# Strong-AI-Lab/ct-vae

Measured on AMD Instinct MI355X. Metric: images/sec/GPU fwd+bwd, 64×64×3 bs=64; recon+KL vs CPU ref, higher is better.
Workload: dtype f32; 1 GPU; VanillaVAE 64x64x3 train step fwd+loss+bwd+Adam (configs/vae.yaml shapes at the batch BASELINE.json's metric names, bs=64, on one MI355X; BASELINE.json configs[1..4] are the `configs` entries); per_gpu_batch=64, global_batch=64, latent_dim=128, parallelism=single, hipgraph=True, allreduce_overlap=False

## Files before the change

### ct-vae_amd/csrc/api.hip

```cpp
#include "../../include/ctvae_hip.h"

#include "common.hpp"
#include "gatlayer.hpp"
#include "glinear.hpp"
#include "pair.hpp"

namespace ctvae {
int launch_tapgemm(const ConvGeom& g, const float* G, const float* W, const float* bias, const float* add,
                   const float* mask, int mask_act, float* S, int act, float* bn_part, float* ws, size_t ws_floats,
                   hipStream_t st, const BnBwdFuse* bnb = nullptr, const InXform* xf = nullptr,
                   const WinoFilters* wf = nullptr, SplitKRaw* raw = nullptr, int out_pix = 0);
bool out_pix_supported(const ConvGeom& g, size_t ws_floats, int out_pix);
bool wino_supported(const ConvGeom& g, size_t ws_floats);
bool wino_enabled();
int wino_set_enabled(int on);
int launch_crop_resize_u8(const unsigned char* img, const long long* rows, float* out, int B, int N, int H, int W, int crop,
                          int S, hipStream_t st);
bool thin_forward_supported(const ConvGeom& g);
bool thin_wgrad_supported(const ConvGeom& g);
int tapgemm_bnb_rows(const ConvGeom& g, size_t ws_floats);
bool img_dgrad_supported(const ConvGeom& g);
void tapgemm_plan(const ConvGeom& g, size_t ws_floats, TapGemmPlan& p);
int launch_wgrad(const ConvGeom& g, const float* X, const float* dY, float* dW, float* dbias, float* ws, size_t ws_bytes,
                 int accumulate, hipStream_t st, const InXform* xf = nullptr, const DyXform* dyx = nullptr);
// ... 265 lines not shown
int ctvae_conv_bn_act_apply_is_separate(int kind, int B, int H, int W, int Ci, int Co, int k, int stride, int pad, int out_pad,
                                        size_t ws_bytes) {
  if (!conv_kind_ok(kind)) return 0;
  ConvGeom g;
  if (conv_geom(g, kind, 0, B, H, W, Ci, Co, k, stride, pad, out_pad)) return 0;
  TapGemmPlan plan;
  tapgemm_plan(g, ws_bytes / sizeof(float), plan);
  return (plan.splitk > 1 && bn_fused_ok(g.B * g.sH * g.sW, Co)) ? 0 : 1;
}

int ctvae_conv_bn_act_forward(int kind, const float* x, const float* w, const float* bias, const float* gamma,
                              const float* beta, float* running_mean, float* running_var, float momentum, float eps,
                              int training, int act, float* y, float* a_out, float* save_mean, float* save_invstd,
                              float* scale_shift_out, int64_t* num_batches_tracked, int B, int H, int W, int Ci, int Co, int k,
                              int stride, int pad, int out_pad, const float* in_scale, const float* in_shift, int in_act,
                              float* ws, size_t ws_bytes, void* stream) {
  long long* nbt = (long long*)num_batches_tracked;
  if (!x || !w || !gamma || !beta || !y || !ws || !conv_kind_ok(kind)) return kErrBadArg;
  if ((in_scale != nullptr) != (in_shift != nullptr)) return kErrBadArg;
  if (in_scale != nullptr && !ctvae_conv_input_transform_supported(kind, B, H, W, Ci, Co, k, stride, pad, out_pad)) return kErrBadArg;
  const InXform xf{in_scale, in_shift, in_act};
  const InXform* xfp = in_scale != nullptr ? &xf : nullptr;
  if (!a_out && !scale_shift_out) return kErrBadArg;
  if (training && (!save_mean || !save_invstd)) return kErrBadArg;
  if (!training && (!running_mean || !running_var)) return kErrBadArg;
  if (Co % 4 != 0) return kErrBadArg;
  ConvGeom g;
  if (conv_geom(g, kind, 0, B, H, W, Ci, Co, k, stride, pad, out_pad)) return kErrBadArg;
  const size_t wsf = ws_bytes / sizeof(float);
  TapGemmPlan plan;
  tapgemm_plan(g, wsf, plan);
  const int R = g.B * g.sH * g.sW;
  if (plan.splitk > 1 || !training) {
    SplitKRaw raw{ws, 0};
    const bool fused = training && plan.splitk > 1 && bn_fused_ok(R, Co);
    int rc = launch_tapgemm(g, x, w, bias, nullptr, nullptr, 0, y, ACT_NONE, nullptr, ws, wsf, (hipStream_t)stream, nullptr, xfp,
                            nullptr, fused ? &raw : nullptr);
    if (rc) return rc;
    if (raw.splitk > 1) {
      const BnFusedFwd p{ws, row_map_of(g), raw.splitk, R, Co, bias, gamma, beta, running_mean, running_var, momentum, eps, save_mean, save_invstd,
                         scale_shift_out, nbt, y, a_out, act};
      return launch_bn_fused_forward(p, (hipStream_t)stream);
    }
    return launch_bn_forward(y, R, Co, gamma, beta, running_mean, running_var, momentum, eps, training, act, a_out, save_mean,
                             save_invstd, ws, ws_bytes, nbt, (hipStream_t)stream, scale_shift_out);
  }
  const int nparts = plan.bn_parts;
  if (wsf < bn_workspace_floats(Co, nparts)) return kErrWorkspace;
  int rc = launch_tapgemm(g, x, w, bias, nullptr, nullptr, 0, y, ACT_NONE, ws, nullptr, 0, (hipStream_t)stream, nullptr, xfp);
  if (rc) return rc;
  return launch_bn_finish_forward(y, R, Co, nparts, gamma, beta, running_mean, running_var, momentum, eps, training, act,
                                  a_out, save_mean, save_invstd, ws, nbt, (hipStream_t)stream, scale_shift_out);
}

int ctvae_conv_dgrad(int kind, const float* dy, const float* w, const float* add, const float* mask, int mask_act,
                     float* dx, int B, int H, int W, int Ci, int Co, int k, int stride, int pad, int out_pad,
// ... 151 lines not shown
  return pl.splitk;
}

int ctvae_conv_backward_lazy(int kind, const float* x, const float* dy, const float* w, float* dw, float* dbias, float* dx_slices,
                             int B, int H, int W, int Ci, int Co, int k, int stride, int pad, int out_pad, int accumulate,
                             const float* in_scale, const float* in_shift, int in_act, int pixel_major, float* ws, size_t ws_bytes,
                             void* stream) {
  if (!dx_slices) return kErrBadArg;
  g_lazy_pixel_major = pixel_major;
  return conv_backward_impl(kind, x, dy, w, dw, dbias, nullptr, B, H, W, Ci, Co, k, stride, pad, out_pad, accumulate, nullptr, 0,
                            nullptr, nullptr, nullptr, nullptr, nullptr, nullptr, 0, nullptr, 0, nullptr, nullptr, nullptr, 0, in_scale,
                            in_shift, in_act, nullptr, nullptr, 0, nullptr, ws, ws_bytes, stream, dx_slices);
}

int ctvae_bn_backward_fused(const float* g_a_slices, int slices, int kind, int B, int H, int W, int Ci, int Co, int k, int stride,
                            int pad, int out_pad, const float* y, const float* gamma, const float* beta, const float* save_mean,
                            const float* save_invstd, int act, float* g_y, float* dgamma, float* dbeta, int accumulate, void* stream) {
  if (!g_a_slices || slices < 1 || !y || !gamma || !beta || !save_mean || !save_invstd || !g_y || !dgamma || !dbeta) return kErrBadArg;
  if (!conv_kind_ok(kind)) return kErrBadArg;
  ConvGeom g;
  if (conv_geom(g, kind, 2, B, H, W, Ci, Co, k, stride, pad, out_pad)) return kErrBadArg;
  const BnFusedBwd p{g_a_slices, row_map_of(g), slices, B * H * W, Ci, y, gamma, beta, save_mean, save_invstd, act, g_y, dgamma,
                     dbeta, accumulate};
  return launch_bn_fused_backward(p, (hipStream_t)stream);
}

int ctvae_conv_wgrad_bn_apply_supported(int kind, int B, int H, int W, int Ci, int Co, int k, int stride, int pad, int out_pad) {
  if (!conv_kind_ok(kind)) return 0;
  ConvGeom g;
  if (conv_geom(g, kind, 0, B, H, W, Ci, Co, k, stride, pad, out_pad)) return 0;
  if (upconv_wgrad_supported(g)) return 1;
  return img_enc_supported(g) ? 2 : 0;
}

int ctvae_bn_forward(const float* y, int R, int C, const float* gamma, const float* beta, float* running_mean,
                     float* running_var, float momentum, float eps, int training, int act, float* out,
                     float* save_mean, float* save_invstd, int64_t* num_batches_tracked, float* ws, size_t ws_bytes,
                     void* stream) {
  if (!y || !gamma || !beta || !out || !ws) return kErrBadArg;
// ... 559 lines not shown
```

### ct-vae_amd/csrc/bn.hip

```cpp
#include "common.hpp"
#include "phase.hpp"
#include "finish.hpp"
#include "prof.hpp"

namespace ctvae {
__device__ __forceinline__ float act_dt(float t, int act, float slope) {
  return act == ACT_TANH ? act_bwd_from_out(act_fwd(t, ACT_TANH), ACT_TANH) : act_slope_bwd(t, slope);
}


constexpr int kBnMaxBlocks = 2048;

__device__ __forceinline__ void chan_merge(float& n, float& mean, float& m2, float nb, float mb, float qb) {
  if (nb > 0.f) {
    const float nt = n + nb, d = mb - mean;
    mean += d * (nb / nt);
    m2 += qb + d * d * (n * nb / nt);
    n = nt;
  }
}

__global__ __launch_bounds__(256) void bn_stats_partial_kernel(const float* __restrict__ y, float* __restrict__ part,
                                                               int R, int C, int rows_per_block) {
  __shared__ float sm[256 * 9];
// ... 499 lines not shown
__device__ __forceinline__ int fused_group(int id, int C, int cpw) {
  const int slots = 32 / cpw, lines = C / 32;
  if (lines % 8 != 0) return id;
  const int x = id & 7, t = id >> 3, slot = t % slots, jh = t / slots;
  return (jh * 8 + x) * slots + slot;
}

template <int TPB, int CPW, int SU>
__global__ __launch_bounds__(TPB) void bn_fused_fwd_kernel(const BnFusedFwd p) {
  typedef float rowv __attribute__((ext_vector_type(CPW)));
  __shared__ float sm[(TPB / 64) * CPW];
  BNF_PH(0);
  const int tid = threadIdx.x, c0 = fused_group(blockIdx.x, p.C, CPW) * CPW, R = p.R, C = p.C;
  const int r4 = 4 * tid;
  const bool live = r4 < R;
  float gmv[CPW], btv[CPW], bsv[CPW], rmv[CPW], rvv[CPW];
#pragma unroll
  for (int c = 0; c < CPW; ++c) {
    gmv[c] = p.gamma[c0 + c];
    btv[c] = p.beta[c0 + c];
    bsv[c] = p.bias != nullptr ? p.bias[c0 + c] : 0.f;
    rmv[c] = p.running_mean != nullptr ? p.running_mean[c0 + c] : 0.f;
    rvv[c] = p.running_mean != nullptr ? p.running_var[c0 + c] : 0.f;
  }
  const long long nbt0 = (blockIdx.x == 0 && p.nbt != nullptr) ? p.nbt[0] : 0;
  f32x4 v[CPW];
  BNF_PH(1);
  slice_sum4<CPW, SU>(v, p.part + (long)c0 * R + (live ? r4 : 0), R, (long)C * R, p.S);
#pragma unroll
  for (int c = 0; c < CPW; ++c) v[c] = live ? v[c] + bsv[c] : f32x4{0.f, 0.f, 0.f, 0.f};
  BNF_PH(2);
  float s[CPW];
#pragma unroll
  for (int c = 0; c < CPW; ++c) s[c] = (v[c][0] + v[c][1]) + (v[c][2] + v[c][3]);
  block_sum_n<TPB, CPW>(s, sm);
  BNF_PH(3);
  float mean[CPW], q[CPW];
#pragma unroll
  for (int c = 0; c < CPW; ++c) {
    mean[c] = s[c] / (float)R;
// ... 4 lines not shown
        const float d = v[c][e] - mean[c];
        t += d * d;
      }
    }
    q[c] = t;
  }
  block_sum_n<TPB, CPW>(q, sm);
  BNF_PH(4);
  float sc[CPW], sh[CPW];
#pragma unroll
  for (int c = 0; c < CPW; ++c) {
    const float var = q[c] / (float)R;
    const float invstd = 1.0f / sqrtf(var + p.eps);
    sc[c] = gmv[c] * invstd;
    sh[c] = btv[c] - mean[c] * sc[c];
    if (tid == 0) {
      p.save_mean[c0 + c] = mean[c];
      p.save_invstd[c0 + c] = invstd;
      if (p.scale_shift != nullptr) {
        p.scale_shift[c0 + c] = sc[c];
        p.scale_shift[C + c0 + c] = sh[c];
      }
      if (p.running_mean != nullptr) {
        const float unbiased = R > 1 ? q[c] / (float)(R - 1) : var;
        p.running_mean[c0 + c] = (1.f - p.momentum) * rmv[c] + p.momentum * mean[c];
        p.running_var[c0 + c] = (1.f - p.momentum) * rvv[c] + p.momentum * unbiased;
      }
    }
  }
  if (tid == 0 && blockIdx.x == 0 && p.nbt != nullptr) p.nbt[0] = nbt0 + 1;
  if (live) {
    const bool atanh_ = p.act == ACT_TANH;
    const float asl = act_slope(p.act);
#pragma unroll
    for (int e = 0; e < 4; ++e) {
      rowv yr, ar;
#pragma unroll
      for (int c = 0; c < CPW; ++c) yr[c] = v[c][e];
      if (atanh_) {
#pragma unroll
        for (int c = 0; c < CPW; ++c) ar[c] = act_fwd(yr[c] * sc[c] + sh[c], ACT_TANH);
      } else {
#pragma unroll
        for (int c = 0; c < CPW; ++c) ar[c] = act_slope_fwd(yr[c] * sc[c] + sh[c], asl);
      }
      const long o = (long)row_map_pixel(p.rows, r4 + e) * C + c0;
      *reinterpret_cast<rowv*>(p.y + o) = yr;
      if (p.a != nullptr) *reinterpret_cast<rowv*>(p.a + o) = ar;
    }
  }
#ifdef CTVAE_PHASES
  BNF_PH(5);
  __builtin_amdgcn_s_waitcnt(0);
  BNF_PH(6);
#endif
}

template <int TPB, int CPW, int SU>
__global__ __launch_bounds__(TPB) void bn_fused_bwd_kernel(const BnFusedBwd p) {
  typedef float rowv __attribute__((ext_vector_type(CPW)));
  __shared__ float sm[(TPB / 64) * 2 * CPW];
  BNB_PH(0);
  const int tid = threadIdx.x, c0 = fused_group(blockIdx.x, p.C, CPW) * CPW, R = p.R, C = p.C;
  const int r4 = 4 * tid;
  const bool live = r4 < R;
  rowv yv[4];
  f32x4 g[CPW];
  long po[4];
#pragma unroll
  for (int e = 0; e < 4; ++e) po[e] = live ? (long)row_map_pixel(p.rows, r4 + e) * C + c0 : c0;
#pragma unroll
  for (int e = 0; e < 4; ++e) yv[e] = *reinterpret_cast<const rowv*>(p.y + po[e]);
  float mean[CPW], invstd[CPW], gm[CPW], bt[CPW], s12[2 * CPW], dg0[CPW], db0[CPW];
#pragma unroll
  for (int c = 0; c < CPW; ++c) {
    mean[c] = p.mean[c0 + c]; invstd[c] = p.invstd[c0 + c]; gm[c] = p.gamma[c0 + c]; bt[c] = p.beta[c0 + c];
    dg0[c] = p.accumulate ? p.dgamma[c0 + c] : 0.f;
    db0[c] = p.accumulate ? p.dbeta[c0 + c] : 0.f;
  }
  BNB_PH(1);
  slice_sum4<CPW, SU>(g, p.part + (long)c0 * R + (live ? r4 : 0), R, (long)C * R, p.S);
  BNB_PH(2);
  const bool btanh_ = p.act == ACT_TANH;
  const float bsl_ = act_slope(p.act);
#pragma unroll
  for (int c = 0; c < CPW; ++c) {
    if (!live) g[c] = f32x4{0.f, 0.f, 0.f, 0.f};
// ... 8 lines not shown
      s2 += gp * xh;
    }
    s12[c] = s1;
    s12[CPW + c] = s2;
  }
  BNB_PH(3);
  block_sum_n<TPB, 2 * CPW>(s12, sm);
  BNB_PH(4);
  float k1[CPW], k2[CPW], k3[CPW];
#pragma unroll
  for (int c = 0; c < CPW; ++c) {
    const float db = s12[c], dg = s12[CPW + c];
    k1[c] = gm[c] * invstd[c];
    k2[c] = -k1[c] * dg / (float)R * invstd[c];
    k3[c] = -k1[c] * db / (float)R - k2[c] * mean[c];
    if (tid == 0) {
      p.dgamma[c0 + c] = dg0[c] + dg;
      p.dbeta[c0 + c] = db0[c] + db;
    }
  }
  if (live) {
#pragma unroll
    for (int e = 0; e < 4; ++e) {
      rowv o;
#pragma unroll
      for (int c = 0; c < CPW; ++c) o[c] = k1[c] * g[c][e] + k2[c] * yv[e][c] + k3[c];
      *reinterpret_cast<rowv*>(p.gy + po[e]) = o;
    }
  }
#ifdef CTVAE_PHASES
  BNB_PH(5);
  __builtin_amdgcn_s_waitcnt(0);
  BNB_PH(6);
#endif
}

bool bn_fused_ok(int R, int C) {
  constexpr long max_elems = 1L << 20;
  return R > 0 && R % 4 == 0 && C % 4 == 0 && R <= 4096 && (long)R * C <= max_elems;
}

constexpr int kBnFusedTwoBelow = 256;

#define CTVAE_BN_FUSED_LAUNCH(KERNEL, P, ST)                                                                      \
  do {                                                                                                            \
    const bool two = (P).C < kBnFusedTwoBelow;                                                                    \
    const dim3 grid((P).C / (two ? 2 : 4));                                                                       \
    if ((P).R <= 256) {                                                                                           \
      if (two) hipLaunchKernelGGL((KERNEL<64, 2, 8>), grid, dim3(64), 0, ST, P);                                  \
      else hipLaunchKernelGGL((KERNEL<64, 4, 8>), grid, dim3(64), 0, ST, P);                                      \
    } else if ((P).R <= 1024) {                                                                                   \
      if (two) hipLaunchKernelGGL((KERNEL<256, 2, 8>), grid, dim3(256), 0, ST, P);                                \
      else hipLaunchKernelGGL((KERNEL<256, 4, 8>), grid, dim3(256), 0, ST, P);                                    \
    } else {                                                                                                      \
      if (two) hipLaunchKernelGGL((KERNEL<1024, 2, 4>), grid, dim3(1024), 0, ST, P);                              \
      else hipLaunchKernelGGL((KERNEL<1024, 4, 4>), grid, dim3(1024), 0, ST, P);                                  \
    }                                                                                                             \
  } while (0)

int launch_bn_fused_forward(const BnFusedFwd& p, hipStream_t st) {
  if (!bn_fused_ok(p.R, p.C) || p.S < 1) return kErrBadArg;
  ProfScope ps("bn_fused_fwd_kernel", st, 0.0, 4.0 * (double)p.R * p.C * (p.S + (p.a != nullptr ? 2 : 1)));
  CTVAE_BN_FUSED_LAUNCH(bn_fused_fwd_kernel, p, st);
  CTVAE_LAUNCH_CHECK();
  return 0;
}

int launch_bn_fused_backward(const BnFusedBwd& p, hipStream_t st) {
  if (!bn_fused_ok(p.R, p.C) || p.S < 1) return kErrBadArg;
  ProfScope ps("bn_fused_bwd_kernel", st, 0.0, 4.0 * (double)p.R * p.C * (p.S + 2));
  CTVAE_BN_FUSED_LAUNCH(bn_fused_bwd_kernel, p, st);
  CTVAE_LAUNCH_CHECK();
  return 0;
}

static bool bn_shape_ok(int R, int C) {
  if (C % 4 != 0 || R <= 0) return false;
  const int Q = C / 4;
  return Q >= 256 ? (Q % 256 == 0) : (256 % Q == 0);
}

static int stat_blocks(int R, int C, int* rows_per_block) {
  const int Q = C / 4;
  const int rl = Q >= 256 ? 1 : 256 / Q;
  int nb = R / (rl * 8);
  if (nb < 1) nb = 1;
// ... 131 lines not shown
```

### ct-vae_amd/csrc/finish.hpp

```cpp
#pragma once
#include "common.hpp"

namespace ctvae {

struct ReduceJob {
  const float* part;
  float* dst;
  long n;
  int S;
  long stride;
  int small;
  int vec;
};

struct SplitKJob {
  const float* part;
  int splitk;
  long stride;
  const float* bias;
  const float* add;
  const float* mask;
  int mask_act, act;
  float* S;
  long n4;
// ... 76 lines not shown
  }
}

struct BnFusedFwd {
  const float* part;
  RowMap rows;
  int S, R, C;
  const float *bias, *gamma, *beta;
  float *running_mean, *running_var;
  float momentum, eps;
  float *save_mean, *save_invstd, *scale_shift;
  long long* nbt;
  float* y;
  float* a;
  int act;
};


struct BnFusedBwd {
  const float* part;
  RowMap rows;
  int S, R, C;
  const float *y, *gamma, *beta, *mean, *invstd;
  int act;
  float* gy;
  float *dgamma, *dbeta;
  int accumulate;
};


bool bn_fused_ok(int R, int C);
int launch_bn_fused_forward(const BnFusedFwd& p, hipStream_t st);
int launch_bn_fused_backward(const BnFusedBwd& p, hipStream_t st);

}
```

### ct-vae_amd/kernels.py

```python
import math
import weakref
from dataclasses import dataclass

import torch
from torch.autograd import Function

from . import native

ACT_NONE, ACT_LRELU, ACT_RELU, ACT_TANH = 0, 1, 2, 3
CONV, CONVT = 0, 1
CONV_FLAT = CONV | 0x100
BN_MOMENTUM, BN_EPS = 0.1, 1e-5


@dataclass(frozen=True)
class ConvSpec:
    kind: int
    ci: int
    co: int
    k: int
    stride: int = 1
    pad: int = 0
    out_pad: int = 0
    act: int = ACT_NONE
# ... 669 lines not shown
        if g_out is None:
            return (None,) * 6
        spec3, spec1 = ctx.specs
        w3, w1 = ctx.w
        x, h, out = ctx.saved_tensors
        g_out = _c(g_out)
        g_pre = act_backward_raw(g_out, out, spec1.act) if spec1.act != ACT_NONE else g_out
        g_h = conv_backward_raw(h, g_pre, w1, None, spec1, mask=h, mask_act=spec3.act)
        conv_wgrad_raw(x, g_h, w3, None, spec3)
        g_x = None
        if ctx.needs_input_grad[0]:
            g_x = conv_dgrad_raw(g_h, w3, spec3, (x.shape[1], x.shape[2]), add=g_pre, wino_filters=ctx.wino_u)
        return g_x, None, None, None, None, None


def _conv_bn_act_forward(x, params, running, training, spec, bn_act, lazy_in, want_a, want_coef):
    w, b, gamma, beta = params
    running_mean, running_var, num_batches_tracked = running
    B, H, W, _ = x.shape
    ho, wo = spec.out_hw(H, W)
    C = spec.co
    y = torch.empty((B, ho, wo, C), dtype=torch.float32, device=x.device)
    a = torch.empty_like(y) if want_a else None
    coef = torch.empty(2 * C, dtype=torch.float32, device=x.device) if want_coef else None
    save_mean = torch.empty(C, dtype=torch.float32, device=x.device)
    save_invstd = torch.empty(C, dtype=torch.float32, device=x.device)
    ws = native.workspace(x.device)
    in_coef, in_act = lazy_in if lazy_in is not None else (None, ACT_NONE)
    g = spec.geom(B, H, W)
    native.call("ctvae_conv_bn_act_forward", g[0], x.data_ptr(), w.data_ptr(), native.ptr(b), gamma.data_ptr(),
                beta.data_ptr(), native.ptr(running_mean), native.ptr(running_var), BN_MOMENTUM, BN_EPS,
                1 if training else 0, bn_act, y.data_ptr(), native.ptr(a), save_mean.data_ptr(), save_invstd.data_ptr(),
                native.ptr(coef), native.ptr(num_batches_tracked) if training else None, *g[1:],
                *_coef_ptrs(in_coef, spec.ci), in_act, ws.data_ptr(), ws.numel() * 4)
    return y, a, coef, save_mean, save_invstd


def _bn_backward(g_a, y, bn, bn_act, g_y, grads, part=None, rows=0, coef_out=None, coef_in=None):
    gamma, beta, save_mean, save_invstd = bn
    gg, gbt, acc = grads
    B, H, W, C = y.shape
    ws = native.workspace(y.device)
    native.call("ctvae_bn_backward", g_a.data_ptr(), beta.data_ptr(), y.data_ptr(), B * H * W, C, gamma.data_ptr(),
                save_mean.data_ptr(), save_invstd.data_ptr(), bn_act, native.ptr(g_y), gg.data_ptr(), gbt.data_ptr(), acc,
                native.ptr(part), rows, native.ptr(coef_out), native.ptr(coef_in), ws.data_ptr(), ws.numel() * 4)


class ConvBNAct(Function):

    @staticmethod
    def forward(ctx, x, w, b, gamma, beta, running_mean, running_var, training, spec, bn_act, num_batches_tracked=None,
                lazy_out=False):
        global _last_link
        _req_cuda(x, w, gamma)
        ctx.link_in = link_of(x)
        ctx.x_slices_ok = bool(getattr(x, "_ctvae_grad_slices_ok", False))
        lazy_in = getattr(x, "_ctvae_lazy_bn", None) if x.is_contiguous() else None
        x = _c(x)
        y, a, coef, save_mean, save_invstd = _conv_bn_act_forward(
            x, (w, b, gamma, beta), (running_mean, running_var, num_batches_tracked), training, spec, bn_act, lazy_in,
            want_a=not lazy_out, want_coef=lazy_out)
        ctx.spec, ctx.bn_act, ctx.training = spec, bn_act, training
        ctx.params = (w, b, gamma, beta)
        ctx.lazy_in = lazy_in
        ctx.save_for_backward(x, y, save_mean, save_invstd)
        ctx.link_out = _last_link = BNLink(y, save_mean, save_invstd, gamma, beta, bn_act) if training else None
        if lazy_out:
            global _last_lazy
            _last_lazy = (coef, bn_act)
            return y
        return a

    @staticmethod
    def backward(ctx, g_a):
        if not ctx.training:
            raise RuntimeError("backward through eval-mode BatchNorm is not supported on the HIP path")
        spec = ctx.spec
        w, b, gamma, beta = ctx.params
        x, y, save_mean, save_invstd = ctx.saved_tensors
        g_a = _c(g_a)
        in_coef, in_act = ctx.lazy_in if ctx.lazy_in is not None else (None, ACT_NONE)
        gg, gbt, accg = _grad_targets(gamma, beta)
        lazy = ctx.link_out.take_lazy(g_a) if ctx.link_out is not None else None
        if lazy is not None:
            g_y = torch.empty_like(y)
            native.call("ctvae_bn_backward_fused", lazy[0].data_ptr(), lazy[1], *lazy[2], y.data_ptr(), gamma.data_ptr(),
                        beta.data_ptr(), save_mean.data_ptr(), save_invstd.data_ptr(), ctx.bn_act, g_y.data_ptr(), gg.data_ptr(),
                        gbt.data_ptr(), accg)
        else:
            part, rows, coef = ctx.link_out.take(g_a) if ctx.link_out is not None else (None, 0, None)
            if coef is not None:
                part, rows = None, 0
                if not ctx.needs_input_grad[0] and wgrad_bn_apply_mode(spec, x.shape[0], x.shape[1], x.shape[2]) == 2:
                    conv_wgrad_raw(x, g_a, w, b, spec, dy_bn=(y, coef, ctx.bn_act, None), bn_commit=(gg, gbt, accg))
                    return (None,) * 12
            g_y = torch.empty_like(y)
            _bn_backward(g_a, y, (gamma, beta, save_mean, save_invstd), ctx.bn_act, g_y, (gg, gbt, accg), part, rows, coef_in=coef)
        g_x = wgrad_then_dgrad(x, g_y, w, b, spec, ctx.needs_input_grad[0], ctx.link_in, in_coef=in_coef, in_act=in_act,
                               grad_slices=ctx.x_slices_ok)
        return (g_x,) + (None,) * 11


# ... 5 lines not shown
    return int(_geom_query("ctvae_conv_wgrad_bn_apply_supported", spec.geom(B, H, W)))


def wgrad_bn_apply_supported(spec: ConvSpec, B, H, W) -> bool:
    return wgrad_bn_apply_mode(spec, B, H, W) == 1


class ConvBNActConvAct(Function):

    @staticmethod
    def forward(ctx, x, w1, b1, gamma, beta, running_mean, running_var, num_batches_tracked, w2, b2, training, spec1, spec2, bn_act):
        _req_cuda(x, w1, w2, gamma)
        ctx.link_in = link_of(x)
        lazy_in = ctx.lazy_in = getattr(x, "_ctvae_lazy_bn", None) if x.is_contiguous() else None
        x = _c(x)
        y1, _, coef, save_mean, save_invstd = _conv_bn_act_forward(
            x, (w1, b1, gamma, beta), (running_mean, running_var, num_batches_tracked), training, spec1, bn_act, lazy_in,
            want_a=False, want_coef=True)
        r = conv_forward_raw(y1, w2, b2, spec2, in_coef=coef, in_act=bn_act)
        ctx.act_out = offer_out_act_link(r, spec2.act) if (training and spec2.act != ACT_NONE) else None
        ctx.specs, ctx.bn_act, ctx.training = (spec1, spec2), bn_act, training
        ctx.params = (w1, b1, gamma, beta, w2, b2)
        ctx.save_for_backward(x, y1, r, coef, save_mean, save_invstd)
        return r

    @staticmethod
    def backward(ctx, g_r):
        if not ctx.training:
            raise RuntimeError("backward through eval-mode BatchNorm is not supported on the HIP path")
        spec1, spec2 = ctx.specs
        w1, b1, gamma, beta, w2, b2 = ctx.params
# ... 1392 lines not shown
```

### ct-vae_amd/native.py

```python
import ctypes
import os

import torch

_HERE = os.path.dirname(os.path.abspath(__file__))
LIB_PATH = os.environ.get("CTVAE_LIB_OVERRIDE") or os.path.join(_HERE, "lib", "libctvae_hip.so")

_c = ctypes
_fp, _vp, _i, _l, _f, _sz = _c.c_void_p, _c.c_void_p, _c.c_int, _c.c_long, _c.c_float, _c.c_size_t

SIGNATURES = {
    "ctvae_linear_pixmajor_supported": [_i, _i, _i, _i, _sz],
    "ctvae_linear_pixmajor_forward": [_fp, _fp, _fp, _fp, _i, _i, _i, _i, _i, _fp, _sz, _vp],
    "ctvae_conv_forward": [_i, _fp, _fp, _fp, _fp, _fp] + [_i] * 10 + [_fp, _fp, _i, _fp, _fp, _fp, _sz, _vp],
    "ctvae_wino_filters_batch": [_i, _vp, _vp, _vp, _vp, _vp, _vp],
    "ctvae_conv_bn_act_forward": [_i, _fp, _fp, _fp, _fp, _fp, _fp, _fp, _f, _f, _i, _i, _fp, _fp, _fp, _fp, _fp, _fp] + [_i] * 9
                                 + [_fp, _fp, _i, _fp, _sz, _vp],
    "ctvae_conv_dgrad": [_i, _fp, _fp, _fp, _fp, _i, _fp] + [_i] * 9 + [_fp, _fp, _sz, _vp],
    "ctvae_conv_wgrad": [_i, _fp, _fp, _fp, _fp] + [_i] * 10 + [_fp, _fp, _i, _fp, _fp, _i, _fp, _fp, _fp, _i, _fp, _sz, _vp],
    "ctvae_conv_backward": [_i, _fp, _fp, _fp, _fp, _fp, _fp] + [_i] * 10 + [_fp, _i, _fp, _fp, _fp, _fp, _fp, _fp, _i, _fp, _i,
                            _fp, _fp, _fp, _i, _fp, _fp, _i, _fp, _fp, _i, _fp, _fp, _sz, _vp],
    "ctvae_conv_backward_lazy": [_i, _fp, _fp, _fp, _fp, _fp, _fp] + [_i] * 10 + [_fp, _fp, _i, _i, _fp, _sz, _vp],
    "ctvae_bn_backward_fused": [_fp, _i] + [_i] * 10 + [_fp, _fp, _fp, _fp, _fp, _i, _fp, _fp, _fp, _i, _vp],
    "ctvae_bn_forward": [_fp, _i, _i, _fp, _fp, _fp, _fp, _f, _f, _i, _i, _fp, _fp, _fp, _fp, _fp, _sz, _vp],
    "ctvae_bn_backward": [_fp, _fp, _fp, _i, _i, _fp, _fp, _fp, _i, _fp, _fp, _fp, _i, _fp, _i, _fp, _fp, _fp, _sz, _vp],
    "ctvae_permute": [_fp, _fp, _i, _i, _i, _i, _vp],
    "ctvae_crop_resize_u8": [_fp, _fp, _fp, _i, _i, _i, _i, _i, _i, _vp],
    "ctvae_gat_score": [_i, _fp, _fp, _fp, _fp, _fp, _fp, _i, _i, _i, _i, _f, _vp],
    "ctvae_gat_score_backward": [_fp, _fp, _fp, _fp, _fp, _fp, _fp, _fp, _fp, _fp, _i, _i, _i, _i, _f, _vp],
    "ctvae_gat_layer_forward": [_fp, _fp, _i, _fp, _fp, _fp, _fp, _fp, _fp, _i, _fp, _i, _i, _i, _f, _i, _vp],
    "ctvae_gat_layer_backward": [_fp, _fp, _i, _fp, _fp, _fp, _fp, _fp, _fp, _i, _fp, _fp, _fp, _fp, _fp, _fp, _i, _fp, _fp, _fp,
                                 _fp, _i, _i, _i, _i, _f, _i, _vp],
    "ctvae_ct_reg_forward": [_fp, _fp, _fp, _fp, _f, _f, _f, _i, _i, _vp],
    "ctvae_ct_reg_backward": [_fp, _fp, _fp, _fp, _fp, _f, _f, _f, _fp, _fp, _i, _i, _vp],
    "ctvae_ct_blend_softmax_forward": [_fp, _fp, _fp, _l, _i, _i, _vp],
    "ctvae_ct_blend_softmax_backward": [_fp, _fp, _fp, _fp, _fp, _fp, _l, _i, _i, _vp],
    "ctvae_ct_latent_ce_forward": [_fp, _fp, _fp, _l, _i, _vp],
    "ctvae_ct_latent_ce_backward": [_fp, _fp, _fp, _fp, _l, _i, _vp],
# ... 72 lines not shown
    "ctvae_defer_begin": [_fp, _sz],
    "ctvae_defer_flush": [_vp],
}
_RESTYPES = {
    "ctvae_version": _c.c_char_p,
    "ctvae_arch": _c.c_char_p,
    "ctvae_error_string": _c.c_char_p,
    "ctvae_workspace_bytes": _c.c_size_t,
    "ctvae_prof_enable": None,
    "ctvae_prof_calibrate": None,
    "ctvae_prof_report": _c.c_size_t,
    "ctvae_conv_backward_bn_rows": _c.c_int,
    "ctvae_conv_backward_lazy_slices": _c.c_int,
    "ctvae_conv_forward_lazy_slices": _c.c_int,
    "ctvae_conv_bn_act_apply_is_separate": _c.c_int,
    "ctvae_winograd_enable": _c.c_int,
    "ctvae_conv_wino_filter_floats": _c.c_size_t,
    "ctvae_dip_state_floats": _c.c_size_t,
    "ctvae_adam_state_floats": _c.c_size_t,
    "ctvae_grad_clip_workspace_floats": _c.c_size_t,
    "ctvae_mssim_part_floats": _c.c_size_t,
    "ctvae_glinear_wgrad_ws_bytes": _c.c_size_t,
    "ctvae_conv_input_transform_supported": _c.c_int,
    "ctvae_conv_wgrad_bn_apply_supported": _c.c_int,
}
EXPORTS = sorted(list(SIGNATURES) + list(_RESTYPES))

_lib = None


# ... 15 lines not shown
            raise RuntimeError(f"{LIB_PATH} does not export {name} (stale build?)")
        fn.argtypes = argtypes
        fn.restype = _c.c_int
    for name, res in _RESTYPES.items():
        fn = getattr(lib, name, None)
        if fn is None:
            raise RuntimeError(f"{LIB_PATH} does not export {name} (stale build?)")
        fn.restype = res
        fn.argtypes = {"ctvae_error_string": [_c.c_int], "ctvae_prof_enable": [_c.c_int],
                       "ctvae_prof_calibrate": [_c.c_void_p, _c.c_int],
                       "ctvae_prof_report": [_c.c_char_p, _c.c_size_t],
                       "ctvae_conv_backward_bn_rows": [_c.c_int] * 10 + [_c.c_size_t],
                       "ctvae_conv_backward_lazy_slices": [_c.c_int] * 11 + [_c.c_size_t],
                       "ctvae_conv_forward_lazy_slices": [_c.c_int] * 10 + [_c.c_size_t],
                       "ctvae_conv_bn_act_apply_is_separate": [_c.c_int] * 10 + [_c.c_size_t],
                       "ctvae_winograd_enable": [_c.c_int],
                       "ctvae_dip_state_floats": [_c.c_int, _c.c_int],
                       "ctvae_glinear_wgrad_ws_bytes": [_c.c_int, _c.c_int, _c.c_int],
                       "ctvae_conv_wino_filter_floats": [_c.c_int] * 10 + [_c.c_size_t],
                       "ctvae_conv_input_transform_supported": [_c.c_int] * 10,
                       "ctvae_conv_wgrad_bn_apply_supported": [_c.c_int] * 10}.get(name, [])
    if lib.ctvae_arch() != b"gfx950":
        raise RuntimeError("libctvae_hip.so was not built for gfx950")
    _lib = lib
    return lib


def check(code: int, what: str):
    if code != 0:
        msg = load().ctvae_error_string(int(code)).decode()
# ... 14 lines not shown
def workspace(device) -> torch.Tensor:
    key = (device.index if device.index is not None else torch.cuda.current_device(), torch.cuda.current_stream().cuda_stream)
    ws = _workspaces.get(key)
    if ws is None:
        n = load().ctvae_workspace_bytes()
        ws = torch.empty(n // 4, dtype=torch.float32, device=device)
        _workspaces[key] = ws
    return ws


def call(name: str, *args):
    lib = load()
    check(getattr(lib, name)(*args, stream_ptr()), name)


_wino_on = None


def winograd_enable(on: bool) -> bool:
    global _wino_on
    prev = bool(load().ctvae_winograd_enable(1 if on else 0))
    _wino_on = bool(on)
    return prev


def winograd_enabled() -> bool:
    global _wino_on
    if _wino_on is None:
        lib = load()
        _wino_on = bool(lib.ctvae_winograd_enable(1))
# ... 22 lines not shown
```

### include/ctvae_hip.h

```cpp
#ifndef CTVAE_HIP_H
#define CTVAE_HIP_H
#include <stddef.h>
#include <stdint.h>

#ifdef __cplusplus
extern "C" {
#endif

#define CTVAE_ACT_NONE 0
#define CTVAE_ACT_LRELU 1
#define CTVAE_ACT_RELU 2
#define CTVAE_ACT_TANH 3

#define CTVAE_CONV 0
#define CTVAE_CONVT 1
#define CTVAE_W_CI_TAP 0x100

const char* ctvae_version(void);
const char* ctvae_arch(void);
const char* ctvae_error_string(int code);
size_t ctvae_workspace_bytes(void);

int ctvae_conv_forward(int kind, const float* x, const float* w, const float* bias, const float* add, float* y, int B,
                       int H, int W, int Ci, int Co, int k, int stride, int pad, int out_pad, int act, const float* in_scale,
// ... 4 lines not shown
                                  float* ws, size_t ws_bytes, void* stream);
int ctvae_wino_filters_batch(int n, const float* const* w, float* const* fwd_filters, float* const* dgrad_filters, const int* Ci,
                             const int* Co, void* stream);
size_t ctvae_conv_wino_filter_floats(int kind, int B, int H, int W, int Ci, int Co, int k, int stride, int pad, int out_pad,
                                     size_t ws_bytes);
int ctvae_conv_input_transform_supported(int kind, int B, int H, int W, int Ci, int Co, int k, int stride, int pad,
                                         int out_pad);

int ctvae_conv_bn_act_apply_is_separate(int kind, int B, int H, int W, int Ci, int Co, int k, int stride, int pad, int out_pad,
                                        size_t ws_bytes);
int ctvae_conv_bn_act_forward(int kind, const float* x, const float* w, const float* bias, const float* gamma,
                              const float* beta, float* running_mean, float* running_var, float momentum, float eps,
                              int training, int act, float* y, float* a_out, float* save_mean, float* save_invstd,
                              float* scale_shift_out, int64_t* num_batches_tracked, int B, int H, int W, int Ci, int Co, int k,
                              int stride, int pad, int out_pad, const float* in_scale, const float* in_shift, int in_act,
                              float* ws, size_t ws_bytes, void* stream);

int ctvae_conv_dgrad(int kind, const float* dy, const float* w, const float* add, const float* mask, int mask_act,
                     float* dx, int B, int H, int W, int Ci, int Co, int k, int stride, int pad, int out_pad,
                     const float* wino_filters, float* ws, size_t ws_bytes, void* stream);

int ctvae_conv_wgrad(int kind, const float* x, const float* dy, float* dw, float* dbias, int B, int H, int W, int Ci,
                     int Co, int k, int stride, int pad, int out_pad, int accumulate, const float* in_scale,
                     const float* in_shift, int in_act, const float* dy_bn_y, const float* dy_bn_coef, int dy_bn_act,
                     float* gy_out, float* bn_dgamma, float* bn_dbeta, int bn_accumulate, float* ws, size_t ws_bytes,
                     void* stream);
int ctvae_conv_backward_bn_rows(int kind, int B, int H, int W, int Ci, int Co, int k, int stride, int pad, int out_pad,
                                size_t ws_bytes);
int ctvae_conv_backward(int kind, const float* x, const float* dy, const float* w, float* dw, float* dbias, float* dx, int B,
                        int H, int W, int Ci, int Co, int k, int stride, int pad, int out_pad, int accumulate, const float* mask,
                        int mask_act, const float* wino_filters, const float* bn_y, const float* bn_mean,
                        const float* bn_invstd, const float* bn_gamma, const float* bn_beta, int bn_act, float* bn_part,
                        int bn_part_rows, float* bn_coef_out, float* bn_dgamma, float* bn_dbeta, int bn_accumulate,
                        const float* in_scale, const float* in_shift, int in_act,
                        const float* dy_bn_y, const float* dy_bn_coef, int dy_bn_act, float* gy_out, float* ws, size_t ws_bytes,
                        void* stream);

int ctvae_conv_backward_lazy_slices(int kind, int B, int H, int W, int Ci, int Co, int k, int stride, int pad, int out_pad,
                                    int for_bn, size_t ws_bytes);
int ctvae_conv_backward_lazy(int kind, const float* x, const float* dy, const float* w, float* dw, float* dbias, float* dx_slices,
                             int B, int H, int W, int Ci, int Co, int k, int stride, int pad, int out_pad, int accumulate,
                             const float* in_scale, const float* in_shift, int in_act, int pixel_major, float* ws, size_t ws_bytes,
                             void* stream);
int ctvae_bn_backward_fused(const float* g_a_slices, int slices, int kind, int B, int H, int W, int Ci, int Co, int k, int stride,
                            int pad, int out_pad, const float* y, const float* gamma, const float* beta, const float* save_mean,
                            const float* save_invstd, int act, float* g_y, float* dgamma, float* dbeta, int accumulate, void* stream);

int ctvae_conv_wgrad_bn_apply_supported(int kind, int B, int H, int W, int Ci, int Co, int k, int stride, int pad,
                                        int out_pad);

int ctvae_bn_forward(const float* y, int R, int C, const float* gamma, const float* beta, float* running_mean,
                     float* running_var, float momentum, float eps, int training, int act, float* out,
                     float* save_mean, float* save_invstd, int64_t* num_batches_tracked, float* ws, size_t ws_bytes,
                     void* stream);
int ctvae_bn_backward(const float* g_a, const float* beta, const float* y, int R, int C, const float* gamma,
                      const float* save_mean, const float* save_invstd, int act, float* g_y, float* dgamma,
                      float* dbeta, int accumulate, const float* part_in, int part_rows, float* coef_out,
                      const float* coef_in, float* ws, size_t ws_bytes, void* stream);

int ctvae_pair_mlp_forward(const float* u, const float* v, int ld, const float* w2, const float* b2, float* out, int B, int N,
                           int H, float slope, int per_sample, const int32_t* row_of, void* stream);
// ... 218 lines not shown
```

Measured before the change: 88910 images/s.

## Split fused BN kernels across row ranges and keep channel-major y copy for backward

The fused split-K BN forward and backward kernels gain a second grid dimension. Each of several blocks per channel group recomputes the full statistics reduction but writes only its own row range, which raises block count for small-C layers. The forward kernel also writes a channel-major copy of the pre-activation y, so the backward kernel can read y with coalesced vector loads instead of strided pixel-major gathers. The cost is redundant reduction work in every extra block, an extra y write and buffer per layer, and more launch variants.

Result: no change. 89500 images/s, median of 3 (+0.7%).

```diff
diff --git a/ct-vae_amd/csrc/api.hip b/ct-vae_amd/csrc/api.hip
--- a/ct-vae_amd/csrc/api.hip
+++ b/ct-vae_amd/csrc/api.hip
@@ -303,8 +303,9 @@
                               int training, int act, float* y, float* a_out, float* save_mean, float* save_invstd,
                               float* scale_shift_out, int64_t* num_batches_tracked, int B, int H, int W, int Ci, int Co, int k,
                               int stride, int pad, int out_pad, const float* in_scale, const float* in_shift, int in_act,
-                              float* ws, size_t ws_bytes, void* stream) {
+                              float* y_cm_out, int* y_cm_written, float* ws, size_t ws_bytes, void* stream) {
   long long* nbt = (long long*)num_batches_tracked;
+  if (y_cm_written != nullptr) *y_cm_written = 0;
   if (!x || !w || !gamma || !beta || !y || !ws || !conv_kind_ok(kind)) return kErrBadArg;
   if ((in_scale != nullptr) != (in_shift != nullptr)) return kErrBadArg;
   if (in_scale != nullptr && !ctvae_conv_input_transform_supported(kind, B, H, W, Ci, Co, k, stride, pad, out_pad)) return kErrBadArg;
@@ -328,7 +329,8 @@
     if (rc) return rc;
     if (raw.splitk > 1) {
       const BnFusedFwd p{ws, row_map_of(g), raw.splitk, R, Co, bias, gamma, beta, running_mean, running_var, momentum, eps, save_mean, save_invstd,
-                         scale_shift_out, nbt, y, a_out, act};
+                         scale_shift_out, nbt, y, a_out, act, y_cm_out};
+      if (y_cm_written != nullptr && y_cm_out != nullptr) *y_cm_written = 1;
       return launch_bn_fused_forward(p, (hipStream_t)stream);
     }
     return launch_bn_forward(y, R, Co, gamma, beta, running_mean, running_var, momentum, eps, training, act, a_out, save_mean,
@@ -510,15 +512,23 @@
 }
 
 int ctvae_bn_backward_fused(const float* g_a_slices, int slices, int kind, int B, int H, int W, int Ci, int Co, int k, int stride,
-                            int pad, int out_pad, const float* y, const float* gamma, const float* beta, const float* save_mean,
-                            const float* save_invstd, int act, float* g_y, float* dgamma, float* dbeta, int accumulate, void* stream) {
+                            int pad, int out_pad, const float* y, const float* y_cm, const float* gamma, const float* beta,
+                            const float* save_mean, const float* save_invstd, int act, float* g_y, float* dgamma, float* dbeta,
+                            int accumulate, void* stream) {
   if (!g_a_slices || slices < 1 || !y || !gamma || !beta || !save_mean || !save_invstd || !g_y || !dgamma || !dbeta) return kErrBadArg;
   if (!conv_kind_ok(kind)) return kErrBadArg;
   ConvGeom g;
   if (conv_geom(g, kind, 2, B, H, W, Ci, Co, k, stride, pad, out_pad)) return kErrBadArg;
   const BnFusedBwd p{g_a_slices, row_map_of(g), slices, B * H * W, Ci, y, gamma, beta, save_mean, save_invstd, act, g_y, dgamma,
-                     dbeta, accumulate};
+                     dbeta, accumulate, y_cm};
   return launch_bn_fused_backward(p, (hipStream_t)stream);
+}
+
+int ctvae_bn_owner_plan(int R, int C, int* plan_out) {
+  BnOwnerPlan pl;
+  if (!plan_out || !bn_owner_plan(R, C, pl)) return kErrBadArg;
+  plan_out[0] = pl.tpb; plan_out[1] = pl.cpw; plan_out[2] = pl.q; plan_out[3] = 4 * pl.tpr; plan_out[4] = pl.grid_cap;
+  return 0;
 }
 
 int ctvae_conv_wgrad_bn_apply_supported(int kind, int B, int H, int W, int Ci, int Co, int k, int stride, int pad, int out_pad) {
diff --git a/ct-vae_amd/csrc/bn.hip b/ct-vae_amd/csrc/bn.hip
--- a/ct-vae_amd/csrc/bn.hip
+++ b/ct-vae_amd/csrc/bn.hip
@@ -537,6 +537,8 @@
   const int tid = threadIdx.x, c0 = fused_group(blockIdx.x, p.C, CPW) * CPW, R = p.R, C = p.C;
   const int r4 = 4 * tid;
   const bool live = r4 < R;
+  const int rq = blockIdx.y;
+  const bool mine = live && tid >= rq * p.tpr && tid < (rq + 1) * p.tpr;
   float gmv[CPW], btv[CPW], bsv[CPW], rmv[CPW], rvv[CPW];
 #pragma unroll
   for (int c = 0; c < CPW; ++c) {
@@ -546,7 +548,7 @@
     rmv[c] = p.running_mean != nullptr ? p.running_mean[c0 + c] : 0.f;
     rvv[c] = p.running_mean != nullptr ? p.running_var[c0 + c] : 0.f;
   }
-  const long long nbt0 = (blockIdx.x == 0 && p.nbt != nullptr) ? p.nbt[0] : 0;
+  const long long nbt0 = (blockIdx.x == 0 && rq == 0 && p.nbt != nullptr) ? p.nbt[0] : 0;
   f32x4 v[CPW];
   BNF_PH(1);
   slice_sum4<CPW, SU>(v, p.part + (long)c0 * R + (live ? r4 : 0), R, (long)C * R, p.S);
@@ -581,7 +583,7 @@
     const float invstd = 1.0f / sqrtf(var + p.eps);
     sc[c] = gmv[c] * invstd;
     sh[c] = btv[c] - mean[c] * sc[c];
-    if (tid == 0) {
+    if (tid == 0 && rq == 0) {
       p.save_mean[c0 + c] = mean[c];
       p.save_invstd[c0 + c] = invstd;
       if (p.scale_shift != nullptr) {
@@ -595,8 +597,8 @@
       }
     }
   }
-  if (tid == 0 && blockIdx.x == 0 && p.nbt != nullptr) p.nbt[0] = nbt0 + 1;
-  if (live) {
+  if (tid == 0 && blockIdx.x == 0 && rq == 0 && p.nbt != nullptr) p.nbt[0] = nbt0 + 1;
+  if (mine) {
     const bool atanh_ = p.act == ACT_TANH;
     const float asl = act_slope(p.act);
 #pragma unroll
@@ -611,9 +613,18 @@
 #pragma unroll
         for (int c = 0; c < CPW; ++c) ar[c] = act_slope_fwd(yr[c] * sc[c] + sh[c], asl);
       }
-      const long o = (long)row_map_pixel(p.rows, r4 + e) * C + c0;
+      const int px = row_map_pixel(p.rows, r4 + e);
+      const long o = (long)px * C + c0;
       *reinterpret_cast<rowv*>(p.y + o) = yr;
       if (p.a != nullptr) *reinterpret_cast<rowv*>(p.a + o) = ar;
+      if (p.ycm != nullptr && p.rows.ncls != 1) {
+#pragma unroll
+        for (int c = 0; c < CPW; ++c) p.ycm[(long)(c0 + c) * R + px] = yr[c];
+      }
+    }
+    if (p.ycm != nullptr && p.rows.ncls == 1) {
+#pragma unroll
+      for (int c = 0; c < CPW; ++c) *reinterpret_cast<f32x4*>(p.ycm + (long)(c0 + c) * R + r4) = v[c];
     }
   }
 #ifdef CTVAE_PHASES
@@ -623,7 +634,7 @@
 #endif
 }
 
-template <int TPB, int CPW, int SU>
+template <int TPB, int CPW, int SU, bool YCM>
 __global__ __launch_bounds__(TPB) void bn_fused_bwd_kernel(const BnFusedBwd p) {
   typedef float rowv __attribute__((ext_vector_type(CPW)));
   __shared__ float sm[(TPB / 64) * 2 * CPW];
@@ -631,13 +642,31 @@
   const int tid = threadIdx.x, c0 = fused_group(blockIdx.x, p.C, CPW) * CPW, R = p.R, C = p.C;
   const int r4 = 4 * tid;
   const bool live = r4 < R;
+  const int rq = blockIdx.y;
+  const bool mine = live && tid >= rq * p.tpr && tid < (rq + 1) * p.tpr;
   rowv yv[4];
   f32x4 g[CPW];
-  long po[4];
-#pragma unroll
-  for (int e = 0; e < 4; ++e) po[e] = live ? (long)row_map_pixel(p.rows, r4 + e) * C + c0 : c0;
-#pragma unroll
-  for (int e = 0; e < 4; ++e) yv[e] = *reinterpret_cast<const rowv*>(p.y + po[e]);
+  int px[4];
+#pragma unroll
+  for (int e = 0; e < 4; ++e) px[e] = live ? row_map_pixel(p.rows, r4 + e) : 0;
+  if constexpr (YCM) {
+    if (p.rows.ncls == 1) {
+#pragma unroll
+      for (int c = 0; c < CPW; ++c) {
+        const f32x4 t = *reinterpret_cast<const f32x4*>(p.ycm + (long)(c0 + c) * R + (live ? r4 : 0));
+#pragma unroll
+        for (int e = 0; e < 4; ++e) yv[e][c] = t[e];
+      }
+    } else {
+#pragma unroll
+      for (int e = 0; e < 4; ++e)
+#pragma unroll
+        for (int c = 0; c < CPW; ++c) yv[e][c] = p.ycm[(long)(c0 + c) * R + px[e]];
+    }
+  } else {
+#pragma unroll
+    for (int e = 0; e < 4; ++e) yv[e] = *reinterpret_cast<const rowv*>(p.y + (long)px[e] * C + c0);
+  }
   float mean[CPW], invstd[CPW], gm[CPW], bt[CPW], s12[2 * CPW], dg0[CPW], db0[CPW];
 #pragma unroll
   for (int c = 0; c < CPW; ++c) {
@@ -676,18 +705,18 @@
     k1[c] = gm[c] * invstd[c];
     k2[c] = -k1[c] * dg / (float)R * invstd[c];
     k3[c] = -k1[c] * db / (float)R - k2[c] * mean[c];
-    if (tid == 0) {
+    if (tid == 0 && rq == 0) {
       p.dgamma[c0 + c] = dg0[c] + dg;
       p.dbeta[c0 + c] = db0[c] + db;
     }
   }
-  if (live) {
+  if (mine) {
 #pragma unroll
     for (int e = 0; e < 4; ++e) {
       rowv o;
 #pragma unroll
       for (int c = 0; c < CPW; ++c) o[c] = k1[c] * g[c][e] + k2[c] * yv[e][c] + k3[c];
-      *reinterpret_cast<rowv*>(p.gy + po[e]) = o;
+      *reinterpret_cast<rowv*>(p.gy + (long)px[e] * C + c0) = o;
     }
   }
 #ifdef CTVAE_PHASES
@@ -703,35 +732,59 @@
 }
 
 constexpr int kBnFusedTwoBelow = 256;
-
-#define CTVAE_BN_FUSED_LAUNCH(KERNEL, P, ST)                                                                      \
+constexpr int kBnOwnerGridCap = 256;
+constexpr int kBnOwnerMinRange = 128;
+
+bool bn_owner_plan(int R, int C, BnOwnerPlan& pl) {
+  if (!bn_fused_ok(R, C)) return false;
+  pl.tpb = R <= 256 ? 64 : (R <= 1024 ? 256 : 1024);
+  pl.cpw = C < kBnFusedTwoBelow ? 2 : 4;
+  const int groups = C / pl.cpw, nthr = R / 4;
+  int q = kBnOwnerGridCap / groups;
+  if (q > nthr / kBnOwnerMinRange) q = nthr / kBnOwnerMinRange;
+  if (q < 1) q = 1;
+  pl.tpr = (ceil_div(nthr, q) + 63) / 64 * 64;
+  pl.q = ceil_div(nthr, pl.tpr);
+  if (pl.q == 1) pl.tpr = pl.tpb;
+  pl.grid_cap = groups > kBnOwnerGridCap ? groups : kBnOwnerGridCap;
+  return true;
+}
+
+#define CTVAE_BN_FUSED_LAUNCH(KERNEL, P, PL, ST, ...)                                                             \
   do {                                                                                                            \
-    const bool two = (P).C < kBnFusedTwoBelow;                                                                    \
-    const dim3 grid((P).C / (two ? 2 : 4));                                                                       \
-    if ((P).R <= 256) {                                                                                           \
-      if (two) hipLaunchKernelGGL((KERNEL<64, 2, 8>), grid, dim3(64), 0, ST, P);                                  \
-      else hipLaunchKernelGGL((KERNEL<64, 4, 8>), grid, dim3(64), 0, ST, P);                                      \
-    } else if ((P).R <= 1024) {                                                                                   \
-      if (two) hipLaunchKernelGGL((KERNEL<256, 2, 8>), grid, dim3(256), 0, ST, P);                                \
-      else hipLaunchKernelGGL((KERNEL<256, 4, 8>), grid, dim3(256), 0, ST, P);                                    \
+    const bool two = (PL).cpw == 2;                                                                               \
+    const dim3 grid((P).C / (PL).cpw, (PL).q);                                                                    \
+    if ((PL).tpb == 64) {                                                                                         \
+      if (two) hipLaunchKernelGGL((KERNEL<64, 2, 8 __VA_ARGS__>), grid, dim3(64), 0, ST, P);                      \
+      else hipLaunchKernelGGL((KERNEL<64, 4, 8 __VA_ARGS__>), grid, dim3(64), 0, ST, P);                          \
+    } else if ((PL).tpb == 256) {                                                                                 \
+      if (two) hipLaunchKernelGGL((KERNEL<256, 2, 8 __VA_ARGS__>), grid, dim3(256), 0, ST, P);                    \
+      else hipLaunchKernelGGL((KERNEL<256, 4, 8 __VA_ARGS__>), grid, dim3(256), 0, ST, P);                        \
     } else {                                                                                                      \
-      if (two) hipLaunchKernelGGL((KERNEL<1024, 2, 4>), grid, dim3(1024), 0, ST, P);                              \
-      else hipLaunchKernelGGL((KERNEL<1024, 4, 4>), grid, dim3(1024), 0, ST, P);                                  \
+      if (two) hipLaunchKernelGGL((KERNEL<1024, 2, 4 __VA_ARGS__>), grid, dim3(1024), 0, ST, P);                  \
+      else hipLaunchKernelGGL((KERNEL<1024, 4, 4 __VA_ARGS__>), grid, dim3(1024), 0, ST, P);                      \
     }                                                                                                             \
   } while (0)
-
-int launch_bn_fused_forward(const BnFusedFwd& p, hipStream_t st) {
-  if (!bn_fused_ok(p.R, p.C) || p.S < 1) return kErrBadArg;
-  ProfScope ps("bn_fused_fwd_kernel", st, 0.0, 4.0 * (double)p.R * p.C * (p.S + (p.a != nullptr ? 2 : 1)));
-  CTVAE_BN_FUSED_LAUNCH(bn_fused_fwd_kernel, p, st);
+#define CTVAE_COMMA ,
+
+int launch_bn_fused_forward(BnFusedFwd p, hipStream_t st) {
+  BnOwnerPlan pl;
+  if (!bn_owner_plan(p.R, p.C, pl) || p.S < 1) return kErrBadArg;
+  p.tpr = pl.tpr;
+  ProfScope ps("bn_fused_fwd_kernel", st, 0.0, 4.0 * (double)p.R * p.C * (p.S + (p.a != nullptr ? 2 : 1) + (p.ycm != nullptr ? 1 : 0)));
+  CTVAE_BN_FUSED_LAUNCH(bn_fused_fwd_kernel, p, pl, st);
   CTVAE_LAUNCH_CHECK();
   return 0;
 }
 
-int launch_bn_fused_backward(const BnFusedBwd& p, hipStream_t st) {
-  if (!bn_fused_ok(p.R, p.C) || p.S < 1) return kErrBadArg;
+int launch_bn_fused_backward(BnFusedBwd p, hipStream_t st) {
+  BnOwnerPlan pl;
+  if (!bn_owner_plan(p.R, p.C, pl) || p.S < 1) return kErrBadArg;
+  if (p.ycm == nullptr) { pl.q = 1; pl.tpr = pl.tpb; }
+  p.tpr = pl.tpr;
   ProfScope ps("bn_fused_bwd_kernel", st, 0.0, 4.0 * (double)p.R * p.C * (p.S + 2));
-  CTVAE_BN_FUSED_LAUNCH(bn_fused_bwd_kernel, p, st);
+  if (p.ycm != nullptr) CTVAE_BN_FUSED_LAUNCH(bn_fused_bwd_kernel, p, pl, st, CTVAE_COMMA true);
+  else CTVAE_BN_FUSED_LAUNCH(bn_fused_bwd_kernel, p, pl, st, CTVAE_COMMA false);
   CTVAE_LAUNCH_CHECK();
   return 0;
 }
diff --git a/ct-vae_amd/csrc/finish.hpp b/ct-vae_amd/csrc/finish.hpp
--- a/ct-vae_amd/csrc/finish.hpp
+++ b/ct-vae_amd/csrc/finish.hpp
@@ -114,6 +114,8 @@
   float* y;
   float* a;
   int act;
+  float* ycm = nullptr;
+  int tpr = 0;
 };
 
 
@@ -126,11 +128,17 @@
   float* gy;
   float *dgamma, *dbeta;
   int accumulate;
+  const float* ycm = nullptr;
+  int tpr = 0;
 };
 
+struct BnOwnerPlan {
+  int tpb, cpw, q, tpr, grid_cap;
+};
 
 bool bn_fused_ok(int R, int C);
-int launch_bn_fused_forward(const BnFusedFwd& p, hipStream_t st);
-int launch_bn_fused_backward(const BnFusedBwd& p, hipStream_t st);
+bool bn_owner_plan(int R, int C, BnOwnerPlan& pl);
+int launch_bn_fused_forward(BnFusedFwd p, hipStream_t st);
+int launch_bn_fused_backward(BnFusedBwd p, hipStream_t st);
 
 }
diff --git a/ct-vae_amd/kernels.py b/ct-vae_amd/kernels.py
--- a/ct-vae_amd/kernels.py
+++ b/ct-vae_amd/kernels.py
@@ -1,3 +1,4 @@
+import ctypes
 import math
 import weakref
 from dataclasses import dataclass
@@ -707,7 +708,7 @@
         return g_x, None, None, None, None, None
 
 
-def _conv_bn_act_forward(x, params, running, training, spec, bn_act, lazy_in, want_a, want_coef):
+def _conv_bn_act_forward(x, params, running, training, spec, bn_act, lazy_in, want_a, want_coef, want_ycm=False):
     w, b, gamma, beta = params
     running_mean, running_var, num_batches_tracked = running
     B, H, W, _ = x.shape
@@ -721,12 +722,16 @@
     ws = native.workspace(x.device)
     in_coef, in_act = lazy_in if lazy_in is not None else (None, ACT_NONE)
     g = spec.geom(B, H, W)
+    ycm = None
+    if want_ycm and training and not _geom_query("ctvae_conv_bn_act_apply_is_separate", g, ws.numel() * 4):
+        ycm = torch.empty((C, B * ho * wo), dtype=torch.float32, device=x.device)
+    wrote = ctypes.c_int(0)
     native.call("ctvae_conv_bn_act_forward", g[0], x.data_ptr(), w.data_ptr(), native.ptr(b), gamma.data_ptr(),
                 beta.data_ptr(), native.ptr(running_mean), native.ptr(running_var), BN_MOMENTUM, BN_EPS,
                 1 if training else 0, bn_act, y.data_ptr(), native.ptr(a), save_mean.data_ptr(), save_invstd.data_ptr(),
                 native.ptr(coef), native.ptr(num_batches_tracked) if training else None, *g[1:],
-                *_coef_ptrs(in_coef, spec.ci), in_act, ws.data_ptr(), ws.numel() * 4)
-    return y, a, coef, save_mean, save_invstd
+                *_coef_ptrs(in_coef, spec.ci), in_act, native.ptr(ycm), ctypes.addressof(wrote), ws.data_ptr(), ws.numel() * 4)
+    return y, a, coef, save_mean, save_invstd, (ycm if wrote.value else None)
 
 
 def _bn_backward(g_a, y, bn, bn_act, g_y, grads, part=None, rows=0, coef_out=None, coef_in=None):
@@ -750,10 +755,11 @@
         ctx.x_slices_ok = bool(getattr(x, "_ctvae_grad_slices_ok", False))
         lazy_in = getattr(x, "_ctvae_lazy_bn", None) if x.is_contiguous() else None
         x = _c(x)
-        y, a, coef, save_mean, save_invstd = _conv_bn_act_forward(
+        y, a, coef, save_mean, save_invstd, ycm = _conv_bn_act_forward(
             x, (w, b, gamma, beta), (running_mean, running_var, num_batches_tracked), training, spec, bn_act, lazy_in,
-            want_a=not lazy_out, want_coef=lazy_out)
+            want_a=not lazy_out, want_coef=lazy_out, want_ycm=True)
         ctx.spec, ctx.bn_act, ctx.training = spec, bn_act, training
+        ctx.ycm = ycm
         ctx.params = (w, b, gamma, beta)
         ctx.lazy_in = lazy_in
         ctx.save_for_backward(x, y, save_mean, save_invstd)
@@ -777,8 +783,8 @@
         lazy = ctx.link_out.take_lazy(g_a) if ctx.link_out is not None else None
         if lazy is not None:
             g_y = torch.empty_like(y)
-            native.call("ctvae_bn_backward_fused", lazy[0].data_ptr(), lazy[1], *lazy[2], y.data_ptr(), gamma.data_ptr(),
-                        beta.data_ptr(), save_mean.data_ptr(), save_invstd.data_ptr(), ctx.bn_act, g_y.data_ptr(), gg.data_ptr(),
+            native.call("ctvae_bn_backward_fused", lazy[0].data_ptr(), lazy[1], *lazy[2], y.data_ptr(), native.ptr(ctx.ycm),
+                        gamma.data_ptr(), beta.data_ptr(), save_mean.data_ptr(), save_invstd.data_ptr(), ctx.bn_act, g_y.data_ptr(), gg.data_ptr(),
                         gbt.data_ptr(), accg)
         else:
             part, rows, coef = ctx.link_out.take(g_a) if ctx.link_out is not None else (None, 0, None)
@@ -814,7 +820,7 @@
         ctx.link_in = link_of(x)
         lazy_in = ctx.lazy_in = getattr(x, "_ctvae_lazy_bn", None) if x.is_contiguous() else None
         x = _c(x)
-        y1, _, coef, save_mean, save_invstd = _conv_bn_act_forward(
+        y1, _, coef, save_mean, save_invstd, _ = _conv_bn_act_forward(
             x, (w1, b1, gamma, beta), (running_mean, running_var, num_batches_tracked), training, spec1, bn_act, lazy_in,
             want_a=False, want_coef=True)
         r = conv_forward_raw(y1, w2, b2, spec2, in_coef=coef, in_act=bn_act)
diff --git a/ct-vae_amd/native.py b/ct-vae_amd/native.py
--- a/ct-vae_amd/native.py
+++ b/ct-vae_amd/native.py
@@ -15,13 +15,13 @@
     "ctvae_conv_forward": [_i, _fp, _fp, _fp, _fp, _fp] + [_i] * 10 + [_fp, _fp, _i, _fp, _fp, _fp, _sz, _vp],
     "ctvae_wino_filters_batch": [_i, _vp, _vp, _vp, _vp, _vp, _vp],
     "ctvae_conv_bn_act_forward": [_i, _fp, _fp, _fp, _fp, _fp, _fp, _fp, _f, _f, _i, _i, _fp, _fp, _fp, _fp, _fp, _fp] + [_i] * 9
-                                 + [_fp, _fp, _i, _fp, _sz, _vp],
+                                 + [_fp, _fp, _i, _fp, _fp, _fp, _sz, _vp],
     "ctvae_conv_dgrad": [_i, _fp, _fp, _fp, _fp, _i, _fp] + [_i] * 9 + [_fp, _fp, _sz, _vp],
     "ctvae_conv_wgrad": [_i, _fp, _fp, _fp, _fp] + [_i] * 10 + [_fp, _fp, _i, _fp, _fp, _i, _fp, _fp, _fp, _i, _fp, _sz, _vp],
     "ctvae_conv_backward": [_i, _fp, _fp, _fp, _fp, _fp, _fp] + [_i] * 10 + [_fp, _i, _fp, _fp, _fp, _fp, _fp, _fp, _i, _fp, _i,
                             _fp, _fp, _fp, _i, _fp, _fp, _i, _fp, _fp, _i, _fp, _fp, _sz, _vp],
     "ctvae_conv_backward_lazy": [_i, _fp, _fp, _fp, _fp, _fp, _fp] + [_i] * 10 + [_fp, _fp, _i, _i, _fp, _sz, _vp],
-    "ctvae_bn_backward_fused": [_fp, _i] + [_i] * 10 + [_fp, _fp, _fp, _fp, _fp, _i, _fp, _fp, _fp, _i, _vp],
+    "ctvae_bn_backward_fused": [_fp, _i] + [_i] * 10 + [_fp, _fp, _fp, _fp, _fp, _fp, _i, _fp, _fp, _fp, _i, _vp],
     "ctvae_bn_forward": [_fp, _i, _i, _fp, _fp, _fp, _fp, _f, _f, _i, _i, _fp, _fp, _fp, _fp, _fp, _sz, _vp],
     "ctvae_bn_backward": [_fp, _fp, _fp, _i, _i, _fp, _fp, _fp, _i, _fp, _fp, _fp, _i, _fp, _i, _fp, _fp, _fp, _sz, _vp],
     "ctvae_permute": [_fp, _fp, _i, _i, _i, _i, _vp],
@@ -124,6 +124,7 @@
     "ctvae_conv_backward_lazy_slices": _c.c_int,
     "ctvae_conv_forward_lazy_slices": _c.c_int,
     "ctvae_conv_bn_act_apply_is_separate": _c.c_int,
+    "ctvae_bn_owner_plan": _c.c_int,
     "ctvae_winograd_enable": _c.c_int,
     "ctvae_conv_wino_filter_floats": _c.c_size_t,
     "ctvae_dip_state_floats": _c.c_size_t,
@@ -169,6 +170,7 @@
                        "ctvae_conv_backward_lazy_slices": [_c.c_int] * 11 + [_c.c_size_t],
                        "ctvae_conv_forward_lazy_slices": [_c.c_int] * 10 + [_c.c_size_t],
                        "ctvae_conv_bn_act_apply_is_separate": [_c.c_int] * 10 + [_c.c_size_t],
+                       "ctvae_bn_owner_plan": [_c.c_int, _c.c_int, _c.POINTER(_c.c_int)],
                        "ctvae_winograd_enable": [_c.c_int],
                        "ctvae_dip_state_floats": [_c.c_int, _c.c_int],
                        "ctvae_glinear_wgrad_ws_bytes": [_c.c_int, _c.c_int, _c.c_int],
@@ -213,6 +215,13 @@
     check(getattr(lib, name)(*args, stream_ptr()), name)
 
 
+def bn_owner_plan(R: int, C: int):
+    out = (_c.c_int * 5)()
+    if load().ctvae_bn_owner_plan(int(R), int(C), out) != 0:
+        return None
+    return dict(zip(("threads", "channels", "ranges", "rows_per_range", "grid_cap"), (int(v) for v in out)))
+
+
 _wino_on = None
 
 
diff --git a/include/ctvae_hip.h b/include/ctvae_hip.h
--- a/include/ctvae_hip.h
+++ b/include/ctvae_hip.h
@@ -42,7 +42,7 @@
                               int training, int act, float* y, float* a_out, float* save_mean, float* save_invstd,
                               float* scale_shift_out, int64_t* num_batches_tracked, int B, int H, int W, int Ci, int Co, int k,
                               int stride, int pad, int out_pad, const float* in_scale, const float* in_shift, int in_act,
-                              float* ws, size_t ws_bytes, void* stream);
+                              float* y_cm_out, int* y_cm_written, float* ws, size_t ws_bytes, void* stream);
 
 int ctvae_conv_dgrad(int kind, const float* dy, const float* w, const float* add, const float* mask, int mask_act,
                      float* dx, int B, int H, int W, int Ci, int Co, int k, int stride, int pad, int out_pad,
@@ -70,9 +70,11 @@
                              int B, int H, int W, int Ci, int Co, int k, int stride, int pad, int out_pad, int accumulate,
                              const float* in_scale, const float* in_shift, int in_act, int pixel_major, float* ws, size_t ws_bytes,
                              void* stream);
+int ctvae_bn_owner_plan(int R, int C, int* plan_out);
 int ctvae_bn_backward_fused(const float* g_a_slices, int slices, int kind, int B, int H, int W, int Ci, int Co, int k, int stride,
-                            int pad, int out_pad, const float* y, const float* gamma, const float* beta, const float* save_mean,
-                            const float* save_invstd, int act, float* g_y, float* dgamma, float* dbeta, int accumulate, void* stream);
+                            int pad, int out_pad, const float* y, const float* y_cm, const float* gamma, const float* beta,
+                            const float* save_mean, const float* save_invstd, int act, float* g_y, float* dgamma, float* dbeta,
+                            int accumulate, void* stream);
 
 int ctvae_conv_wgrad_bn_apply_supported(int kind, int B, int H, int W, int Ci, int Co, int k, int stride, int pad,
                                         int out_pad);
```
